# jspenmar/slowtv_monodepth

Hardware: AMD Instinct MI355X
Metric: training images/sec (640×192, 3-frame) at 1/2/4/8 MI355X; warp+SSIM HBM GB/s (higher is better)
Workload: dtype f32

## Files before the change

include/smd_hotpath.h:

```cpp
#ifndef SMD_HOTPATH_H
#define SMD_HOTPATH_H

#include <stddef.h>
#include <stdint.h>

#ifdef __cplusplus
extern "C" {
#endif

#define SMD_ABI_VERSION 8

#define SMD_OK 0
#define SMD_E_INVALID (-1)
#define SMD_E_LAUNCH (-2)
#define SMD_E_WORKSPACE (-3)
#define SMD_E_UNSUPPORTED (-4)

#define SMD_USE_MIN 0x1
#define SMD_USE_AUTOMASK 0x2
#define SMD_LOSS_L1 0x4
#define SMD_NEED_K_GRAD 0x8
#define SMD_USE_EDGES 0x10
#define SMD_LOSS_L2 0x20
#define SMD_MASK_EXPLAINABILITY 0x80
// ... 139 lines not shown
size_t smd_conv3x3_thin_workspace_bytes(int B, int C, int h, int w);
int smd_conv3x3_thin_fwd(const float* xp, const float* weight, float* y, int B, int C, int h, int w, void* stream);
int smd_conv3x3_thin_bwd(const float* xp, const float* weight, const float* g_y, float* g_xp, float* g_weight, void* workspace, size_t workspace_bytes,
                         int B, int C, int h, int w, void* stream);

size_t smd_conv3x3_mfma_packed_bytes(int C, int CO, int pieces);
size_t smd_conv3x3_mfma_workspace_bytes(int B, int C, int CO, int h, int w);
int smd_conv3x3_mfma_pack(const float* weight, void* wp_fwd, void* wp_bwd, int C, int CO, int pieces, void* stream);
int smd_conv3x3_mfma_fwd(const void* xp, const void* wp_fwd, void* y, void* workspace, size_t workspace_bytes,
                         int B, int C, int CO, int h, int w, int pieces, void* stream);
int smd_conv3x3_mfma_bwd_data(const void* g_y, const void* wp_bwd, void* g_xp, void* workspace, size_t workspace_bytes,
                              int B, int C, int CO, int h, int w, int pieces, void* stream);
int smd_conv3x3_mfma_bwd_weight(const void* xp, const void* g_y, float* g_weight, void* workspace, size_t workspace_bytes,
                                int B, int C, int CO, int h, int w, int pieces, void* stream);

size_t smd_conv3x3z_mfma_workspace_bytes(int B, int C, int CO, int h, int w);
int smd_conv3x3z_mfma_fwd(const float* x, const void* wp_fwd, float* y, void* workspace, size_t workspace_bytes,
                          int B, int C, int CO, int h, int w, int pieces, void* stream);
int smd_conv3x3z_mfma_bwd_data(const float* g_y, const void* wp_bwd, float* g_x, void* workspace, size_t workspace_bytes,
                               int B, int C, int CO, int h, int w, int pieces, void* stream);
int smd_conv3x3z_mfma_bwd_weight(const float* x, const float* g_y, float* g_weight, void* workspace, size_t workspace_bytes,
                                 int B, int C, int CO, int h, int w, int pieces, void* stream);

size_t smd_conv7x7s2_packed_bytes(int C, int CO);
size_t smd_conv7x7s2_workspace_bytes(int B, int C, int CO, int H, int W);
int smd_conv7x7s2_pack(const float* weight, void* wp, int C, int CO, void* stream);
int smd_conv7x7s2_fwd(const float* x, const void* wp, float* y, int B, int C, int CO, int H, int W, void* stream);
int smd_conv7x7s2_bwd_weight(const float* x, const float* g_y, float* g_weight, void* workspace, size_t workspace_bytes,
                             int B, int C, int CO, int H, int W, void* stream);

size_t smd_bn_workspace_bytes(int N, int C, int HW);
int smd_bn_fwd(const float* x, const float* residual, const float* gamma, const float* beta, float* running_mean, float* running_var,
               float momentum, float eps, int relu, float* y, float* save_mean, float* save_invstd,
               void* workspace, size_t workspace_bytes, int N, int C, int HW, void* stream);
int smd_bn_bwd(const float* x, const float* y, const float* g_y, const float* gamma, const float* save_mean, const float* save_invstd,
               int relu, float* g_x, float* g_residual, float* g_gamma, float* g_beta,
               void* workspace, size_t workspace_bytes, int N, int C, int HW, void* stream);

int smd_maxpool3x3s2_fwd(const float* x, float* y, uint8_t* idx, int N, int C, int H, int W, void* stream);
int smd_maxpool3x3s2_bwd(const float* g_y, const uint8_t* idx, float* g_x, int N, int C, int H, int W, void* stream);

size_t smd_dwconv7x7_workspace_bytes(int C, int H, int W);
int smd_dwconv7x7_fwd(const float* x, const float* weight, const float* bias, float* y, int N, int C, int H, int W, int flip, void* stream);
int smd_dwconv7x7_wrw(const float* x, const float* g_y, float* g_weight, float* g_bias, void* workspace, size_t workspace_bytes,
                      int N, int C, int H, int W, void* stream);

// ... 33 lines not shown
```

slowtv_monodepth_amd/_lib.py:

```python
from __future__ import annotations

import ctypes as C
import os
from pathlib import Path

import torch

__all__ = ['lib', 'call', 'set_knob', 'reset_knobs', 'knob_epoch', 'lib_path', 'FLAGS', 'REGR_FLAGS', 'SEL_MASKED', 'ptr_array', 'int_array', 'i64_array', 'HotpathError', 'Unsupported']

_HERE = Path(__file__).resolve().parent
lib_path = Path(os.environ.get('SMD_HOTPATH_LIB', _HERE/'libsmd_hotpath.so'))

FLAGS = {'use_min': 0x1, 'use_automask': 0x2, 'loss_l1': 0x4, 'need_k_grad': 0x8, 'use_edges': 0x10, 'loss_l2': 0x20, 'packed_ready': 0x40,
         'mask_explainability': 0x80, 'mask_uncertainty': 0x100, 'use_laplacian': 0x200, 'bwd_skip_rows': 0x400, 'edges_ready': 0x800, 'bwd_no_live': 0x1000}
REGR_FLAGS = {'l1': 0x0, 'log_l1': 0x1, 'berhu': 0x2, 'invert': 0x4}
SEL_MASKED = 255
MAX_SCALES = 8
MAX_SUPPORTS = 8

_vp, _i, _f, _sz, _u64 = C.c_void_p, C.c_int, C.c_float, C.c_size_t, C.c_uint64

PROTOTYPES = {
    'smd_last_error': (C.c_char_p, []),
    'smd_abi_version': (_i, []),
# ... 36 lines not shown
    'smd_decoder_glue_workspace_bytes': (_sz, [_i]*4),
    'smd_conv3x3_headn_workspace_bytes': (_sz, [_i]*5),
    'smd_conv3x3_headn_fwd': (_i, [_vp]*4 + [_i]*6 + [_vp]),
    'smd_conv3x3_headn_bwd_data': (_i, [_vp]*4 + [_i]*6 + [_vp]),
    'smd_conv3x3_headn_bwd_wgt': (_i, [_vp]*6 + [_sz] + [_i]*6 + [_vp]),
    'smd_upsample_stack_fwd': (_i, [_vp]*3 + [_i]*5 + [_vp, _vp]),
    'smd_upsample_stack_bwd': (_i, [_vp]*2 + [_i]*5 + [_vp]*3),
    'smd_scale_mean_workspace_bytes': (_sz, [_vp, _i]),
    'smd_scale_mean_fwd': (_i, [_vp]*2 + [_i]*2 + [_vp]*2 + [_sz, _vp]),
    'smd_scale_mean_bwd': (_i, [_vp]*2 + [_i]*2 + [_vp]*3),
    'smd_conv3x3_thin_workspace_bytes': (_sz, [_i]*4),
    'smd_conv3x3_thin_fwd': (_i, [_vp]*3 + [_i]*4 + [_vp]),
    'smd_conv3x3_thin_bwd': (_i, [_vp]*6 + [_sz] + [_i]*4 + [_vp]),
    'smd_conv3x3_mfma_packed_bytes': (_sz, [_i]*3),
    'smd_conv3x3_mfma_workspace_bytes': (_sz, [_i]*5),
    'smd_conv3x3_mfma_pack': (_i, [_vp]*3 + [_i]*3 + [_vp]),
    'smd_conv3x3_mfma_fwd': (_i, [_vp]*4 + [_sz] + [_i]*6 + [_vp]),
    'smd_conv3x3_mfma_bwd_data': (_i, [_vp]*4 + [_sz] + [_i]*6 + [_vp]),
    'smd_conv3x3_mfma_bwd_weight': (_i, [_vp]*4 + [_sz] + [_i]*6 + [_vp]),
    'smd_conv3x3z_mfma_workspace_bytes': (_sz, [_i]*5),
    'smd_conv3x3z_mfma_fwd': (_i, [_vp]*4 + [_sz] + [_i]*6 + [_vp]),
    'smd_conv3x3z_mfma_bwd_data': (_i, [_vp]*4 + [_sz] + [_i]*6 + [_vp]),
    'smd_conv3x3z_mfma_bwd_weight': (_i, [_vp]*4 + [_sz] + [_i]*6 + [_vp]),
    'smd_conv7x7s2_packed_bytes': (_sz, [_i]*2),
    'smd_conv7x7s2_workspace_bytes': (_sz, [_i]*5),
    'smd_conv7x7s2_pack': (_i, [_vp]*2 + [_i]*2 + [_vp]),
    'smd_conv7x7s2_fwd': (_i, [_vp]*3 + [_i]*5 + [_vp]),
    'smd_conv7x7s2_bwd_weight': (_i, [_vp]*4 + [_sz] + [_i]*5 + [_vp]),
    'smd_conv3x3_head_workspace_bytes': (_sz, [_i]*4),
    'smd_conv3x3_head_fwd': (_i, [_vp]*4 + [_i]*5 + [_vp]),
    'smd_conv3x3_head_bwd': (_i, [_vp]*8 + [_sz] + [_i]*5 + [_vp]),
    'smd_elu_pad_fwd': (_i, [_vp]*3 + [_i]*6 + [_vp]),
    'smd_elu_pad_bwd': (_i, [_vp]*6 + [_sz] + [_i]*6 + [_vp]),
    'smd_elu_up_cat_pad_fwd': (_i, [_vp]*4 + [_i]*6 + [_vp]),
    'smd_elu_up_cat_pad_bwd': (_i, [_vp]*7 + [_sz] + [_i]*6 + [_vp]),
    'smd_bn_workspace_bytes': (_sz, [_i, _i, _i]),
    'smd_bn_fwd': (_i, [_vp]*6 + [_f, _f, _i] + [_vp]*4 + [_sz] + [_i]*3 + [_vp]),
    'smd_bn_bwd': (_i, [_vp]*6 + [_i] + [_vp]*5 + [_sz] + [_i]*3 + [_vp]),
    'smd_maxpool3x3s2_fwd': (_i, [_vp]*3 + [_i]*4 + [_vp]),
    'smd_maxpool3x3s2_bwd': (_i, [_vp]*3 + [_i]*4 + [_vp]),
    'smd_dwconv7x7_workspace_bytes': (_sz, [_i]*3),
    'smd_dwconv7x7_fwd': (_i, [_vp]*4 + [_i]*5 + [_vp]),
    'smd_dwconv7x7_wrw': (_i, [_vp]*5 + [_sz] + [_i]*4 + [_vp]),
    'smd_layernorm_cf_workspace_bytes': (_sz, [_i]*3),
    'smd_layernorm_cf_fwd': (_i, [_vp]*4 + [_i] + [_vp]*2 + [_i]*3 + [_f, _vp]),
    'smd_layernorm_cf_bwd': (_i, [_vp]*2 + [_i] + [_vp]*7 + [_sz] + [_i]*3 + [_vp]),
# ... 73 lines not shown
```

slowtv_monodepth_amd/conv_ops.py:

```python
from __future__ import annotations

from collections import namedtuple

import torch

from . import _lib
from ._device import _check, _check_fb, _on, _ptr, _stream, _workspace, call
from .conv_routing import serve

_BF = torch.bfloat16


def _thin_bwd(xp, weight, g_y, want_x, want_w):
    if not (want_x or want_w): return None, None
    B, C, H, W = xp.shape
    g_xp = torch.empty_like(xp) if want_x else None
    g_w = torch.empty_like(weight) if want_w else None
    ws, nbytes = _workspace(xp.device, _lib.lib.smd_conv3x3_thin_workspace_bytes, B, C, H - 2, W - 2, floor=256) if want_w else (None, 0)
    call('smd_conv3x3_thin_bwd', xp.data_ptr(), weight.data_ptr(), g_y.data_ptr(), _ptr(g_xp), _ptr(g_w), _ptr(ws), nbytes, B, C, H - 2, W - 2, _stream())
    return g_xp, g_w


class _Conv3x3Thin(torch.autograd.Function):
    @staticmethod
# ... 113 lines not shown
                return _mfma_launch('bwd_data', zpad, g_y, packed['wb'], g_xp, nws, dims, pieces)
            ref_data = (lambda: _thin_bwd(xp, weight, g_y, True, False)[0]) if thin_ref else (lambda: cb([True, False, False])[0])
            g_xp = serve(('data' + sfx, *dims), run_data, ref_data, eligible=sv.data and sv.sized, force=force)
        if need_w:
            g_w = torch.empty_like(weight)
            run_wgt = lambda: _mfma_launch('bwd_weight', zpad, xp, g_y, g_w, nws, dims, pieces)
            ref_wgt = (lambda: _thin_bwd(xp, weight, g_y, False, True)[1]) if thin_ref else (lambda: cb([False, True, False])[1].float())
            g_w = serve(('wgt' + sfx, *dims), run_wgt, ref_wgt, eligible=sv.wgt and sv.sized, force=force)
        return g_xp, g_w, None, None, None


def conv3x3_mfma(xp, weight, pieces: int = 3):
    return _Conv3x3Wide.apply(xp, weight, int(pieces), True)


def conv3x3_wide(xp, weight):
    return _Conv3x3Wide.apply(xp, weight, 3, False)


def conv3x3_same(x, weight):
    return _Conv3x3Wide.apply(x, weight, 3, False, True)


class _Conv7x7s2Stem(torch.autograd.Function):
    @staticmethod
    def forward(ctx, x, weight):
        x = _check('x', x)
        if x.ndim != 4: raise ValueError(f'expected (B,C,H,W), got {tuple(x.shape)}')
        B, C, H, W = x.shape
        if weight.ndim != 4 or tuple(weight.shape[1:]) != (C, 7, 7): raise ValueError(f'weight: expected (CO,{C},7,7), got {tuple(weight.shape)}')
        CO = weight.shape[0]
        weight = _check('weight', weight, (CO, C, 7, 7))
        ho, wo = (H - 1)//2 + 1, (W - 1)//2 + 1
        served = _lib.lib.smd_conv7x7s2_workspace_bytes(B, C, CO, H, W) > 0
        y = torch.empty((B, CO, ho, wo), device=x.device, dtype=torch.float32)

        def run_mfma():
            wp, _ = _workspace(x.device, _lib.lib.smd_conv7x7s2_packed_bytes, C, CO)
            call('smd_conv7x7s2_pack', weight.data_ptr(), wp.data_ptr(), C, CO, _stream())
            call('smd_conv7x7s2_fwd', x.data_ptr(), wp.data_ptr(), y.data_ptr(), B, C, CO, H, W, _stream())
            return y
        y = serve(('fwd_s', B, C, CO, H, W), run_mfma, lambda: torch.conv2d(x, weight, None, 2, 3), eligible=served)
        ctx.save_for_backward(x, weight)
        ctx.served = served
        return y

# ... 25 lines not shown
```

slowtv_monodepth_amd/conv_routing.py:

```python
from __future__ import annotations

import torch

from ._lib import Unsupported

_MODE = 'auto'
_ROUTES: dict = {}
_AB_WARMUPS, _AB_ROUNDS, _AB_MARGIN = 2, 5, 0.97
_DECLINED = (Unsupported, ValueError)


def set_conv_route(mode: str = 'auto'):
    global _MODE
    if mode not in ('auto', 'mfma', 'miopen'): raise ValueError(mode)
    _MODE = mode
    _ROUTES.clear()


def conv_routes() -> dict:
    return dict(_ROUTES)


_COARSE_W_MAX, _COARSE_C_MIN = 80, 256
_Z_FWD_WGT = [dict(px_min=1000, ch_max=511), dict(px_min=2400)]
STATIC_RULES = {
    'padded': {'fwd': [dict(thin=True), dict(thin=False, px_min=20000, c_co_max=128*64), dict(thin=False, coarse=True, px_min=1000)],
               'data': [dict(thin=True), dict(thin=False, px_min=5000, c_max=256), dict(thin=False, coarse=True, px_min=1000)],
               'wgt': [dict(thin=False, px_min=20000, co_max=64), dict(thin=False, coarse=True, px_min=2400)]},
    'bf16': {'fwd': [dict(thin=True)], 'data': [dict(thin=True)], 'wgt': [dict(thin=True)]},
    'zpad': {'fwd': _Z_FWD_WGT, 'data': [dict(px_min=1000)], 'wgt': _Z_FWD_WGT},
    'stem': {'fwd': [dict(px_min=20000)], 'wgt': [dict(px_min=20000)]},
}
_FAMILY_OF_SUFFIX = {'': 'padded', 'bf16': 'bf16', 'z': 'zpad', 's': 'stem'}
_BOUNDS = {'px_min': lambda v, B, C, CO, h, w: B*h*w >= v,
           'c_max': lambda v, B, C, CO, h, w: C <= v,
           'co_max': lambda v, B, C, CO, h, w: CO <= v,
           'c_co_max': lambda v, B, C, CO, h, w: C*CO <= v,
           'ch_max': lambda v, B, C, CO, h, w: max(C, CO) <= v,
           'thin': lambda v, B, C, CO, h, w: (CO == 16) == v,
           'coarse': lambda v, B, C, CO, h, w: (w <= _COARSE_W_MAX and C >= _COARSE_C_MIN) == v}


def static_rule(op, B, C, CO, h, w) -> bool:
    kind, _, suffix = op.partition('_')
    clauses = STATIC_RULES[_FAMILY_OF_SUFFIX[suffix]][kind]
    return any(all(_BOUNDS[name](v, B, C, CO, h, w) for name, v in clause.items()) for clause in clauses)


_capturing = torch.cuda.is_current_stream_capturing


def _time_interleaved(run_mfma, run_ref, rounds):
    ev = [[torch.cuda.Event(enable_timing=True) for _ in range(3)] for _ in range(rounds)]
    for e in ev:
        e[0].record(); run_mfma(); e[1].record(); run_ref(); e[2].record()
    torch.cuda.synchronize()
    return [e[0].elapsed_time(e[1])*1e3 for e in ev], [e[1].elapsed_time(e[2])*1e3 for e in ev]


def _conv_route(op, B, C, CO, h, w, run_mfma, run_ref) -> bool:
    if _MODE != 'auto': return _MODE == 'mfma'
    key = (op, B, C, CO, h, w)
    r = _ROUTES.get(key)
    if r is None:
        if _capturing(): return static_rule(op, B, C, CO, h, w)
        for _ in range(_AB_WARMUPS): run_mfma(); run_ref()
        us_m, us_r = _time_interleaved(run_mfma, run_ref, _AB_ROUNDS)
        t_m, t_r = sorted(us_m)[_AB_ROUNDS//2], sorted(us_r)[_AB_ROUNDS//2]
# ... 19 lines not shown
```

slowtv_monodepth_amd/csrc/smd_api.hip:

```cpp
#include <limits.h>
#include <stdarg.h>
#include <stdio.h>
#include <stdlib.h>
#include <string.h>
#include <algorithm>

#include "smd_kernels.h"
#include "smd_smooth_dev.h"

namespace {

thread_local char g_err[512] = "";

int fail(int code, const char* fmt, ...) {
  va_list ap;
  va_start(ap, fmt);
  vsnprintf(g_err, sizeof(g_err), fmt, ap);
  va_end(ap);
  return code;
}

int check_launch(hipError_t e, const char* what) {
  if (e != hipSuccess) return fail(SMD_E_LAUNCH, "%s: %s", what, hipGetErrorString(e));
  return SMD_OK;
// ... 871 lines not shown
static int mfma_bwd_weight(bool zpad, const void* x, const void* g_y, float* g_weight, void* workspace, size_t workspace_bytes, int B, int C, int CO, int h, int w, int pieces, void* stream) {
  if (!x || !g_y || !g_weight || !workspace) return fail(SMD_E_INVALID, "null pointer");
  if (int rc = mfma_check(ConvOp::Wgt, zpad, workspace_bytes, B, C, CO, h, w, pieces, conv_two_tiles())) return rc;
  return check_launch(smd::launch_conv_mfma_bwd_wgt(x, g_y, g_weight, (float*)workspace, zpad, B, C, CO, h, w, pieces, (hipStream_t)stream), zpad ? "conv3x3z_mfma_bwd_weight" : "conv3x3_mfma_bwd_weight");
}
int smd_conv3x3_mfma_fwd(const void* xp, const void* wp_fwd, void* y, void* workspace, size_t workspace_bytes, int B, int C, int CO, int h, int w, int pieces, void* stream) {
  return mfma_form(ConvOp::Fwd, false, xp, wp_fwd, y, workspace, workspace_bytes, B, C, CO, h, w, pieces, stream, "conv3x3_mfma_fwd");
}
int smd_conv3x3_mfma_bwd_data(const void* g_y, const void* wp_bwd, void* g_xp, void* workspace, size_t workspace_bytes, int B, int C, int CO, int h, int w, int pieces, void* stream) {
  return mfma_form(ConvOp::Data, false, g_y, wp_bwd, g_xp, workspace, workspace_bytes, B, C, CO, h, w, pieces, stream, "conv3x3_mfma_bwd_data");
}
int smd_conv3x3_mfma_bwd_weight(const void* xp, const void* g_y, float* g_weight, void* workspace, size_t workspace_bytes, int B, int C, int CO, int h, int w, int pieces, void* stream) {
  return mfma_bwd_weight(false, xp, g_y, g_weight, workspace, workspace_bytes, B, C, CO, h, w, pieces, stream);
}
int smd_conv3x3z_mfma_fwd(const float* x, const void* wp_fwd, float* y, void* workspace, size_t workspace_bytes, int B, int C, int CO, int h, int w, int pieces, void* stream) {
  return mfma_form(ConvOp::Fwd, true, x, wp_fwd, y, workspace, workspace_bytes, B, C, CO, h, w, pieces, stream, "conv3x3z_mfma_fwd");
}
int smd_conv3x3z_mfma_bwd_data(const float* g_y, const void* wp_bwd, float* g_x, void* workspace, size_t workspace_bytes, int B, int C, int CO, int h, int w, int pieces, void* stream) {
  return mfma_form(ConvOp::Data, true, g_y, wp_bwd, g_x, workspace, workspace_bytes, B, C, CO, h, w, pieces, stream, "conv3x3z_mfma_bwd_data");
}
int smd_conv3x3z_mfma_bwd_weight(const float* x, const float* g_y, float* g_weight, void* workspace, size_t workspace_bytes, int B, int C, int CO, int h, int w, int pieces, void* stream) {
  return mfma_bwd_weight(true, x, g_y, g_weight, workspace, workspace_bytes, B, C, CO, h, w, pieces, stream);
}
static bool stem_sizes_ok(int B, int C, int H, int W) {
  if (B < 1 || B > 65535 || C < 1 || H < 1 || W < 1) return false;
  const long long ho = (H - 1)/2 + 1, wo = (W - 1)/2 + 1;
  return (long long)C*H*W < (1ll << 31) && 64*ho*wo < (1ll << 31) && (ho + 3)/4 <= 65535;
}
size_t smd_conv7x7s2_packed_bytes(int C, int CO) { return smd::conv_stem_served(C, CO) ? smd::conv_stem_packed_bytes(C) : 0; }
size_t smd_conv7x7s2_workspace_bytes(int B, int C, int CO, int H, int W) {
  if (!smd::conv_stem_served(C, CO) || !stem_sizes_ok(B, C, H, W)) return 0;
  return align256(smd::conv_stem_wgrad_floats(B, C, H, W)*sizeof(float));
}
int smd_conv7x7s2_pack(const float* weight, void* wp, int C, int CO, void* stream) {
  if (!weight || !wp) return fail(SMD_E_INVALID, "null pointer");
  if (!smd::conv_stem_served(C, CO)) return fail(SMD_E_UNSUPPORTED, "the stem kernels serve CO == 64 with C == 3 | 6, not C=%d CO=%d", C, CO);
  return check_launch(smd::launch_conv_stem_pack(weight, wp, C, (hipStream_t)stream), "conv7x7s2_pack");
}
int smd_conv7x7s2_fwd(const float* x, const void* wp, float* y, int B, int C, int CO, int H, int W, void* stream) {
  if (!x || !wp || !y) return fail(SMD_E_INVALID, "null pointer");
  if (!smd::conv_stem_served(C, CO)) return fail(SMD_E_UNSUPPORTED, "the stem kernels serve CO == 64 with C == 3 | 6, not C=%d CO=%d", C, CO);
  if (!stem_sizes_ok(B, C, H, W)) return fail(SMD_E_INVALID, "invalid sizes B=%d C=%d H=%d W=%d", B, C, H, W);
  return check_launch(smd::launch_conv_stem_fwd(x, wp, y, B, C, H, W, (hipStream_t)stream), "conv7x7s2_fwd");
}
int smd_conv7x7s2_bwd_weight(const float* x, const float* g_y, float* g_weight, void* workspace, size_t workspace_bytes,
                             int B, int C, int CO, int H, int W, void* stream) {
// ... 183 lines not shown
```

slowtv_monodepth_amd/csrc/smd_conv_mfma.hip:

```cpp
#include "smd_common.h"
#include "smd_kernels.h"
#include "smd_split_dev.h"
#include <algorithm>
#include <type_traits>

namespace smd {

template <int P> __device__ __forceinline__ void split_pair(unsigned short a, unsigned short b, unsigned (&p)[P]) {
  static_assert(P == 1, "bfloat16 operands have one piece");
  p[0] = (unsigned)a | ((unsigned)b << 16);
}
template <typename T> struct RawOf { typedef float type; };
template <> struct RawOf<bf16> { typedef unsigned short type; };
template <typename T> __device__ __forceinline__ void store_out(T* p, size_t i, float v);
template <> __device__ __forceinline__ void store_out<float>(float* p, size_t i, float v) { p[i] = v; }
template <> __device__ __forceinline__ void store_out<bf16>(bf16* p, size_t i, float v) { p[i] = __float2bfloat16(v); }

template <int P>
__global__ __launch_bounds__(256) void k_conv_pack_w(const float* __restrict__ w, unsigned short* __restrict__ wp_fwd, unsigned short* __restrict__ wp_bwd, int CO, int C) {
  const int idx = blockIdx.x*256 + threadIdx.x;
  if (idx >= CO*C*9) return;
  const int tap = idx % 9, c = (idx/9) % C, co = idx/(9*C);
  unsigned pk[P];
  split_pair<P>(w[idx], 0.f, pk);
// ... 1118 lines not shown
  double* slice = reinterpret_cast<double*>(partial + (size_t)T*n);
  if (G == 1) hipLaunchKernelGGL(k_conv_wgrad_finalize<true>, dim3(ceil_div(n, 64), 1), dim3(256), 0, st, partial, T, 1u, CO, C, slice, g_w);
  else {
    hipLaunchKernelGGL(k_conv_wgrad_finalize<false>, dim3(ceil_div(n, 64), G), dim3(256), 0, st, partial, T, G, CO, C, slice, g_w);
    hipLaunchKernelGGL(k_conv_wgrad_finalize2, dim3(ceil_div(n, 256)), dim3(256), 0, st, slice, G, CO, C, g_w);
  }
  return hipGetLastError();
}
hipError_t launch_conv_mfma_bwd_wgt(const void* xp, const void* gy, float* g_w, float* partial, bool zpad, int B, int C, int CO, int h, int w, int pieces, hipStream_t st) {
  if (zpad) {
    dim3 grid; int rows, spb;
    wgrad_shape(B, C, CO, h, w, grid, rows, spb, true);
#define SMD_CALL(P) hipLaunchKernelGGL((k_conv_wgrad_dma<P, true>), grid, dim3(256), 0, st, (const float*)xp, (const float*)gy, partial, B, C, CO, h, w, rows, spb)
    SMD_BY_PIECES_F32(pieces, SMD_CALL);
#undef SMD_CALL
  } else {
#define SMD_CALL(P, T) launch_wgrad<P, T>(xp, gy, partial, B, C, CO, h, w, st)
    SMD_BY_PIECES(pieces, SMD_CALL);
#undef SMD_CALL
  }
  return wgrad_finalize(g_w, partial, B, C, CO, h, w, zpad || pieces != 1, st);
}

}

#ifdef SMD_CONV_TRACE
extern "C" int smd_debug_conv_trace(unsigned long long* host_out, int blocks) {
  return (int)hipMemcpyFromSymbol(host_out, HIP_SYMBOL(smd::g_conv_trace), (size_t)blocks*40*sizeof(unsigned long long), 0, hipMemcpyDeviceToHost);
}
#endif
```

slowtv_monodepth_amd/csrc/smd_kernels.h:

```cpp
#pragma once
#include <hip/hip_runtime.h>
#include <stddef.h>
#include <stdint.h>

#include "../../include/smd_hotpath.h"

namespace smd {

constexpr int kFwdCols = 62;
constexpr int kBwdCols = 60;
#ifndef SMD_WAVES_PER_BLOCK
#define SMD_WAVES_PER_BLOCK 4
#endif
constexpr int kWavesPerBlock = SMD_WAVES_PER_BLOCK;
#ifndef SMD_SMOOTH_CHUNK
#define SMD_SMOOTH_CHUNK 1024
#endif
constexpr int kSmoothChunk = SMD_SMOOTH_CHUNK;
__host__ __device__ inline int smooth_chunk_px(int n) { return n > 32768 ? kSmoothChunk : 256; }
__host__ __device__ inline int smooth_chunks_of(int n) { return (n + smooth_chunk_px(n) - 1)/smooth_chunk_px(n); }
constexpr int kSmoothCols = 63, kSmoothRows = 8;
__host__ __device__ inline int smooth_units_of(int hs, int ws) { return ((ws + kSmoothCols - 1)/kSmoothCols)*((hs + kSmoothRows - 1)/kSmoothRows); }
constexpr int kSmoothRowsMain = 16;
__host__ __device__ inline int smooth_units_main(int hs, int ws) { return ((ws + kSmoothCols - 1)/kSmoothCols)*((hs + kSmoothRowsMain - 1)/kSmoothRowsMain); }
// ... 207 lines not shown
  int S;
};
int scale_mean_blocks(MeanSet& ms);
hipError_t launch_scale_mean_fwd(MeanSet ms, int mode, float* partial, unsigned* counter, float* loss, hipStream_t st);
hipError_t launch_scale_mean_bwd(MeanSet ms, int mode, const float* g_loss, hipStream_t st);
hipError_t launch_conv_thin_fwd(const float* xp, const float* wgt, float* y, int B, int C, int h, int w, hipStream_t st);
size_t conv_thin_partials(int B, int C, int h, int w);
hipError_t launch_conv_thin_bwd_wgt(const float* xp, const float* gy, float* g_w, float* partial, int B, int C, int h, int w, hipStream_t st);
hipError_t launch_conv_thin_bwd_data(const float* gy, const float* wgt, float* g_xp, int B, int C, int h, int w, hipStream_t st);
enum class ConvOp { Fwd, Data, Wgt };
inline bool conv_mfma_served(ConvOp op, bool zpad, int C, int CO) {
  const bool thin = !zpad && CO == 16 && (C == 16 || C == 32);
  if (op == ConvOp::Fwd) return (C % 16 == 0 && CO % 32 == 0) || thin;
  if (op == ConvOp::Data) return (CO % 16 == 0 && C % 32 == 0) || (thin && C == 16);
  return CO % 32 == 0 || thin;
}
size_t conv_mfma_packed_elems(int C, int CO, int pieces);
size_t conv_mfma_wgrad_partials(bool zpad, int B, int C, int CO, int h, int w);
size_t conv_mfma_split_elems(ConvOp op, bool zpad, int B, int C, int CO, int h, int w, bool two_tiles);
hipError_t launch_conv_mfma_pack(const float* w, void* wp_fwd, void* wp_bwd, int C, int CO, int pieces, hipStream_t st);
hipError_t launch_conv_mfma_fwd(const void* x, const void* wp_fwd, void* y, float* split_ws, bool zpad, int B, int C, int CO, int h, int w, int pieces, bool two_tiles, hipStream_t st);
hipError_t launch_conv_mfma_bwd_data(const void* gy, const void* wp_bwd, void* g_x, float* split_ws, bool zpad, int B, int C, int CO, int h, int w, int pieces, bool two_tiles, hipStream_t st);
hipError_t launch_conv_mfma_bwd_wgt(const void* x, const void* gy, float* g_w, float* partial, bool zpad, int B, int C, int CO, int h, int w, int pieces, hipStream_t st);
bool conv_stem_served(int C, int CO);
size_t conv_stem_packed_bytes(int C);
size_t conv_stem_wgrad_floats(int B, int C, int H, int W);
hipError_t launch_conv_stem_pack(const float* w, void* wp, int C, hipStream_t st);
hipError_t launch_conv_stem_fwd(const float* x, const void* wp, float* y, int B, int C, int H, int W, hipStream_t st);
hipError_t launch_conv_stem_bwd_wgt(const float* x, const float* gy, float* g_w, float* partial, int B, int C, int H, int W, hipStream_t st);
size_t decoder_bias_partials(int B, int C, int h, int w);
hipError_t launch_elu_pad_fwd(const void* x, const float* bias, void* out, int B, int C, int h, int w, int apply_elu, int dt, hipStream_t st);
hipError_t launch_elu_pad_bwd(const void* x, const float* bias, const void* g_out, void* g_x, float* g_bias, float* ws, int B, int C, int h, int w,
                              int apply_elu, int dt, hipStream_t st);
hipError_t launch_elu_up_cat_pad_fwd(const void* a, const float* bias, const void* skip, void* out, int B, int Ca, int Cs, int h, int w, int dt,
                                     hipStream_t st);
hipError_t launch_elu_up_cat_pad_bwd(const void* a, const float* bias, const void* g_out, void* g_a, void* g_skip, float* g_bias, float* ws,
                                     int B, int Ca, int Cs, int h, int w, int dt, hipStream_t st);
int bn_chunks(int N, int HW);
hipError_t launch_bn_fwd(const float* x, const float* residual, const float* gamma, const float* beta, float* running_mean, float* running_var,
                         float momentum, float eps, int relu, float* y, float* save_mean, float* save_invstd, float* ws, int N, int C, int HW,
                         hipStream_t st);
hipError_t launch_bn_bwd(const float* x, const float* y, const float* g_y, const float* gamma, const float* save_mean, const float* save_invstd,
                         int relu, float* g_x, float* g_res, float* g_gamma, float* g_beta, float* ws, int N, int C, int HW, hipStream_t st);
hipError_t launch_maxpool_fwd(const float* x, float* y, uint8_t* idx, size_t planes, int H, int W, hipStream_t st);
hipError_t launch_maxpool_bwd(const float* g_y, const uint8_t* idx, float* g_x, size_t planes, int H, int W, hipStream_t st);
int dwconv_tiles(int H, int W);
// ... 37 lines not shown
```

slowtv_monodepth_amd/functional.py:

```python
from ._device import _stream, call
from .class_ops import _ScaleMean, crop_resize, lane_shift_selftest, photo_error, recon_reduce, regression_loss, scale_mean, upsample_stack, view_synth
from .conv_ops import conv3x3_mfma, conv3x3_same, conv3x3_thin, conv3x3_wide, conv7x7s2_stem
from .conv_routing import _conv_route, conv_routes, set_conv_route
from .geom_ops import intrinsics, inv_intrinsics, pose_matrices
from .net_ops import batch_norm_act, conv3x3_head, conv3x3_headn, dwconv7x7, elu_pad, elu_up_cat_pad, layer_norm_cf, max_pool3x3s2
from .recon_ops import (PreparedFrames, disp_smooth_blurred, disp_smooth_fused, disp_to_depth, gaussian_blur3x3, image_recon_fused, image_recon_fused_disp,
                        image_recon_prep, loss_path_fused, recon_flags, supports_per_pass)
from .row_skip import _RowSkipTuner, dead_tile_shares, dead_wave_shares, row_skip_tuner

__all__ = ['conv3x3_headn', 'upsample_stack', 'scale_mean', 'conv3x3_mfma', 'conv3x3_wide', 'conv3x3_same', 'set_conv_route', 'conv_routes', 'loss_path_fused', 'crop_resize', 'disp_to_depth', 'image_recon_prep', 'PreparedFrames', 'image_recon_fused', 'image_recon_fused_disp', 'disp_smooth_fused', 'view_synth', 'photo_error', 'recon_reduce',
           'lane_shift_selftest', 'recon_flags', 'regression_loss', 'elu_pad', 'elu_up_cat_pad', 'batch_norm_act', 'max_pool3x3s2', 'dwconv7x7', 'layer_norm_cf', 'pose_matrices', 'intrinsics', 'inv_intrinsics',
           'conv3x3_head', 'conv3x3_thin', 'conv7x7s2_stem', 'gaussian_blur3x3', 'disp_smooth_blurred', 'supports_per_pass', 'row_skip_tuner', 'dead_tile_shares', 'dead_wave_shares']
```

slowtv_monodepth_amd/networks/encoders.py:

```python
from __future__ import annotations

import torch
import torch.nn as nn
import torch.nn.functional as F

__all__ = ['create_encoder', 'FeatureInfo', 'ResNetFeatures', 'ConvNeXtFeatures', 'ENCODERS']


class FeatureInfo:
    def __init__(self, channels, reduction): self._c, self._r = list(channels), list(reduction)
    def channels(self): return list(self._c)
    def reduction(self): return list(self._r)


class BatchNormAct2d(nn.BatchNorm2d):
    fused_enabled = True

    def forward(self, x, residual=None, relu: bool = False):
        fused = (self.fused_enabled and x.is_cuda and self.training and x.dtype == torch.float32 and not torch.is_autocast_enabled() and self.affine
                 and self.track_running_stats and self.momentum is not None and x.is_contiguous())
        if not fused:
            y = super().forward(x)
            if residual is not None: y = y + residual
            return F.relu(y, inplace=True) if relu else y
        from .. import functional as HF
        self._pending_batches = getattr(self, '_pending_batches', 0) + 1
        return HF.batch_norm_act(x, self.weight, self.bias, self.running_mean, self.running_var, residual=residual,
                                 momentum=self.momentum, eps=self.eps, relu=relu)

    def flush_counter(self):
        n = getattr(self, '_pending_batches', 0)
        if n and self.num_batches_tracked is not None: self.num_batches_tracked += n
        self._pending_batches = 0

    def _save_to_state_dict(self, destination, prefix, keep_vars):
        self.flush_counter()
        super()._save_to_state_dict(destination, prefix, keep_vars)

    def train(self, mode: bool = True):
        if not mode: self.flush_counter()
        return super().train(mode)


def _conv3x3(conv: nn.Conv2d, x):
    if (conv.stride == (1, 1) and BatchNormAct2d.fused_enabled and x.is_cuda and x.dtype == torch.float32 and conv.weight.dtype == torch.float32
            and not torch.is_autocast_enabled() and x.is_contiguous()):
        from .. import functional as HF
        return HF.conv3x3_same(x, conv.weight)
    return conv(x)


def _stem(conv: nn.Conv2d, x):
    if (BatchNormAct2d.fused_enabled and x.is_cuda and x.dtype == torch.float32 and conv.weight.dtype == torch.float32
            and not torch.is_autocast_enabled() and x.is_contiguous()):
        from .. import functional as HF
        return HF.conv7x7s2_stem(x, conv.weight)
    return conv(x)


class BasicBlock(nn.Module):
    def __init__(self, cin, cout, stride):
        super().__init__()
        self.conv1 = nn.Conv2d(cin, cout, 3, stride, 1, bias=False); self.bn1 = BatchNormAct2d(cout)
        self.conv2 = nn.Conv2d(cout, cout, 3, 1, 1, bias=False); self.bn2 = BatchNormAct2d(cout)
        self.down = None
        if stride != 1 or cin != cout:
            self.down = nn.Sequential(nn.Conv2d(cin, cout, 1, stride, bias=False), BatchNormAct2d(cout))

    def forward(self, x):
        idt = x if self.down is None else self.down(x)
        x = self.bn1(_conv3x3(self.conv1, x), relu=True)
# ... 135 lines not shown
```

Measured before the change: 941.4.

## Add stride-2 3x3 MFMA forward kernel and route encoder downsampling convs

Adds a bf16-split MFMA forward kernel for stride-2 3x3 convolutions. It loads a halo tile into LDS, rearranged into four parity planes, so each tap reads contiguous strided pixels. It double-buffers channel chunks and falls back to split-K with a reduction kernel when the grid is small. The encoder's stride-2 convs now go through a new autograd function whose backward still calls aten. Routing adds an empty strided rule table, so whether the new kernel actually runs depends on the serve/tuning policy; without it the path falls back to torch.conv2d.

```diff
diff --git a/include/smd_hotpath.h b/include/smd_hotpath.h
--- a/include/smd_hotpath.h
+++ b/include/smd_hotpath.h
@@ -185,6 +185,10 @@
 int smd_conv3x3z_mfma_bwd_weight(const float* x, const float* g_y, float* g_weight, void* workspace, size_t workspace_bytes,
                                  int B, int C, int CO, int h, int w, int pieces, void* stream);
 
+size_t smd_conv3x3s2_mfma_workspace_bytes(int B, int C, int CO, int H, int W);
+int smd_conv3x3s2_mfma_fwd(const float* x, const void* wp_fwd, float* y, void* workspace, size_t workspace_bytes,
+                           int B, int C, int CO, int H, int W, int pieces, void* stream);
+
 size_t smd_conv7x7s2_packed_bytes(int C, int CO);
 size_t smd_conv7x7s2_workspace_bytes(int B, int C, int CO, int H, int W);
 int smd_conv7x7s2_pack(const float* weight, void* wp, int C, int CO, void* stream);
diff --git a/slowtv_monodepth_amd/_lib.py b/slowtv_monodepth_amd/_lib.py
--- a/slowtv_monodepth_amd/_lib.py
+++ b/slowtv_monodepth_amd/_lib.py
@@ -82,6 +82,8 @@
     'smd_conv3x3z_mfma_fwd': (_i, [_vp]*4 + [_sz] + [_i]*6 + [_vp]),
     'smd_conv3x3z_mfma_bwd_data': (_i, [_vp]*4 + [_sz] + [_i]*6 + [_vp]),
     'smd_conv3x3z_mfma_bwd_weight': (_i, [_vp]*4 + [_sz] + [_i]*6 + [_vp]),
+    'smd_conv3x3s2_mfma_workspace_bytes': (_sz, [_i]*5),
+    'smd_conv3x3s2_mfma_fwd': (_i, [_vp]*4 + [_sz] + [_i]*6 + [_vp]),
     'smd_conv7x7s2_packed_bytes': (_sz, [_i]*2),
     'smd_conv7x7s2_workspace_bytes': (_sz, [_i]*5),
     'smd_conv7x7s2_pack': (_i, [_vp]*2 + [_i]*2 + [_vp]),
diff --git a/slowtv_monodepth_amd/conv_ops.py b/slowtv_monodepth_amd/conv_ops.py
--- a/slowtv_monodepth_amd/conv_ops.py
+++ b/slowtv_monodepth_amd/conv_ops.py
@@ -159,6 +159,46 @@
     return _Conv3x3Wide.apply(x, weight, 3, False, True)
 
 
+class _Conv3x3S2(torch.autograd.Function):
+    @staticmethod
+    def forward(ctx, x, weight, pieces, force):
+        x = _check('x', x)
+        if x.ndim != 4: raise ValueError(f'expected (B,C,H,W), got {tuple(x.shape)}')
+        B, C, H, W = x.shape
+        if weight.ndim != 4 or tuple(weight.shape[1:]) != (C, 3, 3): raise ValueError(f'weight: expected (CO,{C},3,3), got {tuple(weight.shape)}')
+        CO = weight.shape[0]
+        weight = _check('weight', weight, (CO, C, 3, 3))
+        nws = _lib.lib.smd_conv3x3s2_mfma_workspace_bytes(B, C, CO, H, W)
+        if force and not nws: raise _lib.Unsupported(f'the stride-2 MFMA forward serves C % 16 == 0 with CO % 32 == 0, not C={C} CO={CO} at {H}x{W}')
+        y = torch.empty((B, CO, (H - 1)//2 + 1, (W - 1)//2 + 1), device=x.device, dtype=torch.float32)
+
+        def run_mfma():
+            wf, _ = _mfma_pack(weight, C, CO, pieces, True, False)
+            ws, n = _workspace(x.device, nws, floor=256)
+            call('smd_conv3x3s2_mfma_fwd', x.data_ptr(), wf.data_ptr(), y.data_ptr(), ws.data_ptr(), n, B, C, CO, H, W, pieces, _stream())
+            return y
+        out = serve(('fwd_z2', B, C, CO, H, W), run_mfma, lambda: torch.conv2d(x, weight, None, 2, 1), eligible=nws > 0, force=force)
+        ctx.save_for_backward(x, weight)
+        return out
+
+    @staticmethod
+    def backward(ctx, g_y):
+        x, weight = ctx.saved_tensors
+        _on(x)
+        B, C, H, W = x.shape
+        CO = weight.shape[0]
+        need_x, need_w = ctx.needs_input_grad[0], ctx.needs_input_grad[1]
+        g_y = _check('grad(y)', g_y, (B, CO, (H - 1)//2 + 1, (W - 1)//2 + 1))
+        cb = lambda mask: torch.ops.aten.convolution_backward(g_y, x, weight, None, [2, 2], [1, 1], [1, 1], False, [0, 0], 1, mask)
+        g_x = serve(('data_z2', B, C, CO, H, W), None, lambda: cb([True, False, False])[0], eligible=False) if need_x else None
+        g_w = serve(('wgt_z2', B, C, CO, H, W), None, lambda: cb([False, True, False])[1], eligible=False) if need_w else None
+        return g_x, g_w, None, None
+
+
+def conv3x3s2_same(x, weight, force: bool = False):
+    return _Conv3x3S2.apply(x, weight, 3, bool(force))
+
+
 class _Conv7x7s2Stem(torch.autograd.Function):
     @staticmethod
     def forward(ctx, x, weight):
diff --git a/slowtv_monodepth_amd/conv_routing.py b/slowtv_monodepth_amd/conv_routing.py
--- a/slowtv_monodepth_amd/conv_routing.py
+++ b/slowtv_monodepth_amd/conv_routing.py
@@ -40,10 +40,12 @@
            'thin': lambda v, B, C, CO, h, w: (CO == 16) == v,
            'coarse': lambda v, B, C, CO, h, w: (w <= _COARSE_W_MAX and C >= _COARSE_C_MIN) == v}
 
+STRIDED_RULES = {'fwd': [], 'data': [], 'wgt': []}
+
 
 def static_rule(op, B, C, CO, h, w) -> bool:
     kind, _, suffix = op.partition('_')
-    clauses = STATIC_RULES[_FAMILY_OF_SUFFIX[suffix]][kind]
+    clauses = STRIDED_RULES[kind] if suffix == 'z2' else STATIC_RULES[_FAMILY_OF_SUFFIX[suffix]][kind]
     return any(all(_BOUNDS[name](v, B, C, CO, h, w) for name, v in clause.items()) for clause in clauses)
 
 
diff --git a/slowtv_monodepth_amd/csrc/smd_api.hip b/slowtv_monodepth_amd/csrc/smd_api.hip
--- a/slowtv_monodepth_amd/csrc/smd_api.hip
+++ b/slowtv_monodepth_amd/csrc/smd_api.hip
@@ -917,6 +917,23 @@
 int smd_conv3x3z_mfma_bwd_weight(const float* x, const float* g_y, float* g_weight, void* workspace, size_t workspace_bytes, int B, int C, int CO, int h, int w, int pieces, void* stream) {
   return mfma_bwd_weight(true, x, g_y, g_weight, workspace, workspace_bytes, B, C, CO, h, w, pieces, stream);
 }
+static bool s2_sizes_ok(int B, int C, int CO, int H, int W) {
+  if (B < 1 || C < 1 || CO < 1 || C > 4096 || CO > 4096 || H < 1 || W < 1 || H >= 32768 || W >= 32768) return false;
+  const long long ho = (H - 1)/2 + 1, wo = (W - 1)/2 + 1;
+  return (long long)C*H*W < (1ll << 29) && CO*ho*wo < (1ll << 29) && (long long)B*((ho + 3)/4)*((wo + 31)/32)*((CO + 31)/32)*((C + 15)/16) < (1ll << 30);
+}
+size_t smd_conv3x3s2_mfma_workspace_bytes(int B, int C, int CO, int H, int W) {
+  if (!s2_sizes_ok(B, C, CO, H, W) || !smd::conv_s2_served(C, CO)) return 0;
+  return align256(std::max((size_t)64, smd::conv_s2_split_elems(B, C, CO, H, W))*sizeof(float));
+}
+int smd_conv3x3s2_mfma_fwd(const float* x, const void* wp_fwd, float* y, void* workspace, size_t workspace_bytes, int B, int C, int CO, int H, int W, int pieces, void* stream) {
+  if (!x || !wp_fwd || !y || !workspace) return fail(SMD_E_INVALID, "null pointer");
+  if (pieces != 2 && pieces != 3) return fail(SMD_E_UNSUPPORTED, "the stride-2 form takes float tensors: pieces 2 or 3, not %d", pieces);
+  if (!s2_sizes_ok(B, C, CO, H, W)) return fail(SMD_E_INVALID, "invalid sizes B=%d C=%d CO=%d H=%d W=%d", B, C, CO, H, W);
+  if (!smd::conv_s2_served(C, CO)) return fail(SMD_E_UNSUPPORTED, "the stride-2 forward serves C %% 16 == 0 with CO %% 32 == 0, not C=%d CO=%d", C, CO);
+  if (workspace_bytes < smd_conv3x3s2_mfma_workspace_bytes(B, C, CO, H, W)) return fail(SMD_E_WORKSPACE, "workspace too small");
+  return check_launch(smd::launch_conv_s2_fwd(x, wp_fwd, y, (float*)workspace, B, C, CO, H, W, pieces, (hipStream_t)stream), "conv3x3s2_mfma_fwd");
+}
 static bool stem_sizes_ok(int B, int C, int H, int W) {
   if (B < 1 || B > 65535 || C < 1 || H < 1 || W < 1) return false;
   const long long ho = (H - 1)/2 + 1, wo = (W - 1)/2 + 1;
diff --git a/slowtv_monodepth_amd/csrc/smd_conv_mfma.hip b/slowtv_monodepth_amd/csrc/smd_conv_mfma.hip
--- a/slowtv_monodepth_amd/csrc/smd_conv_mfma.hip
+++ b/slowtv_monodepth_amd/csrc/smd_conv_mfma.hip
@@ -1164,6 +1164,176 @@
   return wgrad_finalize(g_w, partial, B, C, CO, h, w, zpad || pieces != 1, st);
 }
 
+struct S2Tile { static constexpr int TR = 4, TCW = 32, PLH = TR + 1, PLW = TCW + 1, PL = PLH*PLW, NPIX = 4*PL, GH = 2*TR + 1, GW = 2*TCW + 1, GPIX = GH*GW; };
+
+template <int P, int NM>
+__global__ __launch_bounds__(128*NM) void k_conv_s2_mfma(const float* __restrict__ in_, const uint4* __restrict__ wp, float* __restrict__ out,
+                                                         int CK, int M, int hi, int wi, int ho, int wo, int KS, int kc_per_split, size_t split_stride,
+                                                         unsigned gx, unsigned gy, unsigned gz) {
+  using T = S2Tile;
+  constexpr int NPIX = T::NPIX, PL = T::PL, PLW = T::PLW, GW = T::GW, GPIX = T::GPIX, NPROD = n_products(P), NT = 128*NM;
+  constexpr int kBuf = P*NPIX*2;
+  __shared__ uint4 tile[2*kBuf];
+  const int lane = threadIdx.x & 63, wall = __builtin_amdgcn_readfirstlane(threadIdx.x >> 6), ph = wall & 1, mt = wall >> 1, j = lane & 31, g = lane >> 5;
+  const int MG = M/(32*NM);
+  const unsigned nblk = (unsigned)(MG*KS)*gx*gy*gz, per = (nblk + 7)/8;
+  const unsigned lid = (blockIdx.x & 7)*per + (blockIdx.x >> 3);
+  if (lid >= nblk) return;
+  const int mg = (int)(lid % MG)*NM + mt, ks = (lid/MG) % KS;
+  const unsigned tl = lid/(MG*KS);
+  const int x0 = (int)(tl % gx)*T::TCW, y0 = (int)((tl/gx) % gy)*T::TR, b = (int)(tl/(gx*gy));
+  const int KC = CK >> 4, kc0 = ks*kc_per_split, kc1 = min(KC, kc0 + kc_per_split);
+  const size_t plane = (size_t)hi*wi;
+  const float* src = in_ + (size_t)b*CK*plane;
+
+  constexpr int ITEMS = 2*GPIX, TRIPS = (ITEMS + NT - 1)/NT;
+  int pofs[TRIPS];
+#pragma unroll
+  for (int t = 0; t < TRIPS; ++t) {
+    const int item = min(t*NT + (int)threadIdx.x, ITEMS - 1);
+    const int half = item >= GPIX ? 1 : 0, pg = item - half*GPIX;
+    const int py = pg/GW, px = pg - py*GW;
+    const int yy = 2*y0 + py - 1, xx = 2*x0 + px - 1;
+    pofs[t] = (yy >= 0 && yy < hi && xx >= 0 && xx < wi) ? yy*wi + xx : -1;
+  }
+  float v[TRIPS][8];
+  auto request = [&](int kc) {
+#pragma unroll
+    for (int t = 0; t < TRIPS; ++t) {
+      const int item = min(t*NT + (int)threadIdx.x, ITEMS - 1);
+      const int half = item >= GPIX ? 1 : 0;
+      const float* p = src + (size_t)(kc*16 + half*8)*plane + (size_t)max(pofs[t], 0);
+#pragma unroll
+      for (int e = 0; e < 8; ++e) v[t][e] = pofs[t] >= 0 ? p[(size_t)e*plane] : 0.f;
+    }
+  };
+  auto file_trip = [&](int buf, int t) {
+    const int item = t*NT + (int)threadIdx.x;
+    if (item < ITEMS) {
+      const int half = item >= GPIX ? 1 : 0, pg = item - half*GPIX;
+      const int py = pg/GW, px = pg - py*GW;
+      const int pix = ((py & 1)*2 + (px & 1))*PL + (py >> 1)*PLW + (px >> 1);
+      unsigned pk[4][P];
+#pragma unroll
+      for (int q = 0; q < 4; ++q) split_pair<P>(v[t][2*q], v[t][2*q + 1], pk[q]);
+      const int slot = pix*2 + (half ^ ((pix >> 3) & 1));
+#pragma unroll
+      for (int p = 0; p < P; ++p) tile[buf*kBuf + p*NPIX*2 + slot] = uint4{pk[0][p], pk[1][p], pk[2][p], pk[3][p]};
+    }
+  };
+  auto file = [&](int buf) {
+#pragma unroll
+    for (int t = 0; t < TRIPS; ++t) file_trip(buf, t);
+  };
+
+  f32x16 acc[2], lo[2];
+#pragma unroll
+  for (int nt = 0; nt < 2; ++nt)
+#pragma unroll
+    for (int r = 0; r < 16; ++r) { acc[nt][r] = 0.f; lo[nt][r] = 0.f; }
+
+  bf16x8 A[5][P], Bf[2][2][P];
+  const uint4* wq = wp + ((size_t)mg*KC*9*P)*64 + lane;
+  auto fetch_a = [&](bf16x8 (&dst)[P], int kc, int tap) {
+#pragma unroll
+    for (int p = 0; p < P; ++p) dst[p] = as_frag(wq[(size_t)((kc*9 + tap)*P + p)*64]);
+  };
+  auto read_b = [&](bf16x8 (&dst)[2][P], int buf, int tap) {
+    const int ky = tap/3, kx = tap % 3;
+#pragma unroll
+    for (int nt = 0; nt < 2; ++nt) {
+      const int r = 2*ph + nt;
+      const int pix = ((ky & 1)*2 + (kx & 1))*PL + (r + (ky >> 1))*PLW + j + (kx >> 1);
+      const int slot = pix*2 + (g ^ ((pix >> 3) & 1));
+#pragma unroll
+      for (int p = 0; p < P; ++p) dst[nt][p] = as_frag(tile[buf*kBuf + p*NPIX*2 + slot]);
+    }
+  };
+  auto chunk = [&](int kc, int cur, auto more_tag) {
+    constexpr bool MORE = decltype(more_tag)::value;
+    read_b(Bf[0], cur, 0);
+#pragma unroll
+    for (int tap = 0; tap < 9; ++tap) {
+      if (tap < 8) read_b(Bf[(tap + 1) & 1], cur, tap + 1);
+#pragma unroll
+      for (int t = 0; t < NPROD; ++t)
+#pragma unroll
+        for (int nt = 0; nt < 2; ++nt) {
+          if (t == NPROD - 1) acc[nt] = __builtin_amdgcn_mfma_f32_32x32x16_bf16(A[tap % 5][0], Bf[tap & 1][nt][0], acc[nt], 0, 0, 0);
+          else lo[nt] = __builtin_amdgcn_mfma_f32_32x32x16_bf16(A[tap % 5][prod_a(P, t)], Bf[tap & 1][nt][prod_b(P, t)], lo[nt], 0, 0, 0);
+        }
+      if (tap <= 4) fetch_a(A[(tap + 4) % 5], kc, tap + 4);
+      else if (MORE && tap >= 6) fetch_a(A[tap - 6], kc + 1, tap - 6);
+      if (MORE && tap == 8) fetch_a(A[3], kc + 1, 3);
+      if (MORE && tap == 4) request(kc + 1);
+      if (MORE && tap >= 6) {
+#pragma unroll
+        for (int t = 0; t < TRIPS; ++t) if (t*3/TRIPS == tap - 6) file_trip(cur ^ 1, t);
+      }
+      __builtin_amdgcn_sched_barrier(0);
+    }
+    __syncthreads();
+  };
+
+  if (kc0 < kc1) {
+    request(kc0);
+#pragma unroll
+    for (int tap = 0; tap < 4; ++tap) fetch_a(A[tap], kc0, tap);
+    file(0);
+  }
+  __syncthreads();
+  int kc = kc0;
+  for (; kc + 1 < kc1; ++kc) chunk(kc, (kc - kc0) & 1, std::true_type{});
+  if (kc < kc1) chunk(kc, (kc - kc0) & 1, std::false_type{});
+  float* dst = out + (size_t)ks*split_stride;
+#pragma unroll
+  for (int nt = 0; nt < 2; ++nt) {
+    const int y = y0 + 2*ph + nt, x = x0 + j;
+    if (y < ho && x < wo) {
+#pragma unroll
+      for (int rr = 0; rr < 16; ++rr) {
+        const int m = mg*32 + (rr & 3) + 8*(rr >> 2) + 4*g;
+        dst[(((size_t)b*M + m)*ho + y)*wo + x] = acc[nt][rr] + lo[nt][rr];
+      }
+    }
+  }
+}
+
+struct S2Shape { int NM, KS, kcs; unsigned gx, gy, gz; dim3 grid; size_t out_elems; };
+static S2Shape s2_shape(int B, int C, int CO, int H, int W) {
+  S2Shape s;
+  const int ho = (H - 1)/2 + 1, wo = (W - 1)/2 + 1, KC = C >> 4;
+  s.NM = CO % 128 == 0 ? 4 : 1;
+  s.gx = ceil_div(wo, S2Tile::TCW); s.gy = ceil_div(ho, S2Tile::TR); s.gz = B;
+  const long long base = (long long)s.gx*s.gy*s.gz*(CO/(32*s.NM));
+  int ks = 1;
+  if (base < 192) ks = (int)std::min<long long>(std::max(KC/2, 1), (256 + base - 1)/base);
+  s.kcs = ceil_div(KC, ks); s.KS = ceil_div(KC, s.kcs);
+  s.grid = dim3(8*(unsigned)ceil_div(base*s.KS, 8ll));
+  s.out_elems = (size_t)B*CO*ho*wo;
+  return s;
+}
+size_t conv_s2_split_elems(int B, int C, int CO, int H, int W) {
+  const S2Shape s = s2_shape(B, C, CO, H, W);
+  return s.KS > 1 ? (size_t)s.KS*s.out_elems : 0;
+}
+hipError_t launch_conv_s2_fwd(const float* x, const void* wp_fwd, float* y, float* split_ws, int B, int C, int CO, int H, int W, int pieces, hipStream_t st) {
+  const S2Shape s = s2_shape(B, C, CO, H, W);
+  const int ho = (H - 1)/2 + 1, wo = (W - 1)/2 + 1;
+  const uint4* wq = (const uint4*)wp_fwd;
+  float* dst = s.KS > 1 ? split_ws : y;
+#define SMD_CALL(P) do { \
+    if (s.NM == 4) hipLaunchKernelGGL((k_conv_s2_mfma<P, 4>), s.grid, dim3(512), 0, st, x, wq, dst, C, CO, H, W, ho, wo, s.KS, s.kcs, s.out_elems, s.gx, s.gy, s.gz); \
+    else hipLaunchKernelGGL((k_conv_s2_mfma<P, 1>), s.grid, dim3(128), 0, st, x, wq, dst, C, CO, H, W, ho, wo, s.KS, s.kcs, s.out_elems, s.gx, s.gy, s.gz); } while (0)
+  SMD_BY_PIECES_F32(pieces, SMD_CALL);
+#undef SMD_CALL
+  if (s.KS > 1) {
+    const size_t n4 = s.out_elems/4;
+    hipLaunchKernelGGL((k_conv_split_sum<float>), dim3((unsigned)((n4 + 255)/256)), dim3(256), 0, st, split_ws, y, n4, s.KS);
+  }
+  return hipGetLastError();
+}
+
 }
 
 #ifdef SMD_CONV_TRACE
diff --git a/slowtv_monodepth_amd/csrc/smd_kernels.h b/slowtv_monodepth_amd/csrc/smd_kernels.h
--- a/slowtv_monodepth_amd/csrc/smd_kernels.h
+++ b/slowtv_monodepth_amd/csrc/smd_kernels.h
@@ -253,6 +253,9 @@
 hipError_t launch_conv_mfma_fwd(const void* x, const void* wp_fwd, void* y, float* split_ws, bool zpad, int B, int C, int CO, int h, int w, int pieces, bool two_tiles, hipStream_t st);
 hipError_t launch_conv_mfma_bwd_data(const void* gy, const void* wp_bwd, void* g_x, float* split_ws, bool zpad, int B, int C, int CO, int h, int w, int pieces, bool two_tiles, hipStream_t st);
 hipError_t launch_conv_mfma_bwd_wgt(const void* x, const void* gy, float* g_w, float* partial, bool zpad, int B, int C, int CO, int h, int w, int pieces, hipStream_t st);
+inline bool conv_s2_served(int C, int CO) { return C % 16 == 0 && CO % 32 == 0; }
+size_t conv_s2_split_elems(int B, int C, int CO, int H, int W);
+hipError_t launch_conv_s2_fwd(const float* x, const void* wp_fwd, float* y, float* split_ws, int B, int C, int CO, int H, int W, int pieces, hipStream_t st);
 bool conv_stem_served(int C, int CO);
 size_t conv_stem_packed_bytes(int C);
 size_t conv_stem_wgrad_floats(int B, int C, int H, int W);
diff --git a/slowtv_monodepth_amd/functional.py b/slowtv_monodepth_amd/functional.py
--- a/slowtv_monodepth_amd/functional.py
+++ b/slowtv_monodepth_amd/functional.py
@@ -1,6 +1,6 @@
 from ._device import _stream, call
 from .class_ops import _ScaleMean, crop_resize, lane_shift_selftest, photo_error, recon_reduce, regression_loss, scale_mean, upsample_stack, view_synth
-from .conv_ops import conv3x3_mfma, conv3x3_same, conv3x3_thin, conv3x3_wide, conv7x7s2_stem
+from .conv_ops import conv3x3_mfma, conv3x3_same, conv3x3_thin, conv3x3_wide, conv3x3s2_same, conv7x7s2_stem
 from .conv_routing import _conv_route, conv_routes, set_conv_route
 from .geom_ops import intrinsics, inv_intrinsics, pose_matrices
 from .net_ops import batch_norm_act, conv3x3_head, conv3x3_headn, dwconv7x7, elu_pad, elu_up_cat_pad, layer_norm_cf, max_pool3x3s2
@@ -10,4 +10,4 @@
 
 __all__ = ['conv3x3_headn', 'upsample_stack', 'scale_mean', 'conv3x3_mfma', 'conv3x3_wide', 'conv3x3_same', 'set_conv_route', 'conv_routes', 'loss_path_fused', 'crop_resize', 'disp_to_depth', 'image_recon_prep', 'PreparedFrames', 'image_recon_fused', 'image_recon_fused_disp', 'disp_smooth_fused', 'view_synth', 'photo_error', 'recon_reduce',
            'lane_shift_selftest', 'recon_flags', 'regression_loss', 'elu_pad', 'elu_up_cat_pad', 'batch_norm_act', 'max_pool3x3s2', 'dwconv7x7', 'layer_norm_cf', 'pose_matrices', 'intrinsics', 'inv_intrinsics',
-           'conv3x3_head', 'conv3x3_thin', 'conv7x7s2_stem', 'gaussian_blur3x3', 'disp_smooth_blurred', 'supports_per_pass', 'row_skip_tuner', 'dead_tile_shares', 'dead_wave_shares']
+           'conv3x3_head', 'conv3x3_thin', 'conv3x3s2_same', 'conv7x7s2_stem', 'gaussian_blur3x3', 'disp_smooth_blurred', 'supports_per_pass', 'row_skip_tuner', 'dead_tile_shares', 'dead_wave_shares']
diff --git a/slowtv_monodepth_amd/networks/encoders.py b/slowtv_monodepth_amd/networks/encoders.py
--- a/slowtv_monodepth_amd/networks/encoders.py
+++ b/slowtv_monodepth_amd/networks/encoders.py
@@ -43,10 +43,10 @@
 
 
 def _conv3x3(conv: nn.Conv2d, x):
-    if (conv.stride == (1, 1) and BatchNormAct2d.fused_enabled and x.is_cuda and x.dtype == torch.float32 and conv.weight.dtype == torch.float32
+    if (conv.stride in ((1, 1), (2, 2)) and BatchNormAct2d.fused_enabled and x.is_cuda and x.dtype == torch.float32 and conv.weight.dtype == torch.float32
             and not torch.is_autocast_enabled() and x.is_contiguous()):
         from .. import functional as HF
-        return HF.conv3x3_same(x, conv.weight)
+        return (HF.conv3x3_same if conv.stride == (1, 1) else HF.conv3x3s2_same)(x, conv.weight)
     return conv(x)
 
 
```

Result: slower. 871.1 (-7.5%).
